# cure-lab/MotionCraft

Hardware: AMD Instinct MI355X
Metric: sampled SMPL-X frames/sec (196-frame seq, 1000-step DDPM) (higher is better)
Workload: dtype f32

## Files before the change

include/motioncraft_amd.h:

```cpp
#ifndef MOTIONCRAFT_AMD_H
#define MOTIONCRAFT_AMD_H
#include <stdint.h>

#ifdef __cplusplus
extern "C" {
#endif

#define MC_OK 0
#define MC_ERR_ARG 1
#define MC_ERR_HIP 2
#define MC_ERR_STATE 3
#define MC_ERR_NOCONV 4

typedef struct mc_model mc_model;
typedef struct mc_ctx mc_ctx;

typedef struct mc_model_config {
    int32_t input_feats;
    int32_t max_seq_len;
    int32_t latent_dim;
    int32_t num_parts;
    int32_t num_layers;
    int32_t ffn_dim;
    int32_t time_embed_dim;
// ... 137 lines not shown
int mc_op_temporal_attention(const float* mf_dev, const float* tf_dev, const float* mask_dev, float* yt_dev, int32_t b0, int32_t nb,
                             int32_t B, int32_t T, int32_t Nt, int32_t H, int32_t L, int32_t form, int32_t skip_text,
                             const int32_t* twin_flag_dev, void* stream);
enum { MC_ENC_ATTN_LAYER = 0,
       MC_ENC_ATTN_SMALL = 1,
       MC_ENC_ATTN_STREAM = 2 };
int mc_op_enc_ln(const float* x_dev, const float* gamma_dev, const float* beta_dev, float* y_dev, int64_t rows, int32_t L, float eps,
                 int32_t relu, void* stream);
int mc_op_enc_embed_tokens(const int32_t* ids_dev, const float* emb_dev, const float* pos_dev, float* x_dev, int64_t rows, int32_t S,
                           int32_t d, int32_t vocab, void* stream);
int mc_op_enc_attention(const float* qkv_dev, const uint8_t* valid_dev, float* out_dev, int32_t B, int32_t S, int32_t d, int32_t heads,
                        int32_t causal, int32_t form, void* stream);
enum { MC_GM_PLAIN = 0, MC_GM_ENC = 4 };
typedef struct mc_gemm_strided {
    const float* a_dev; int64_t lda, a_gstride;
    const float* w_dev; int64_t ldw, w_gstride;
    const float* bias_dev; int64_t b_gstride;
    float* c_dev; int64_t ldc, c_gstride;
    const float* res_dev; int64_t ldr, r_gstride;
    const float* add_dev; int64_t ld_add, dup_rows;
    int32_t add_mod, act, act_after_res, M, N, K;
} mc_gemm_strided;
int mc_op_gemm_strided(int32_t mode, int32_t groups, const mc_gemm_strided* args, void* stream);
int mc_op_bigru_steps(const float* gi_dev, const float* whh_dev, const float* bhh_dev, float* h_dev, const int32_t* lens_dev,
                      int32_t len_div, int32_t B, int32_t S, int32_t H, int32_t s0, int32_t steps, void* stream);
int mc_op_conv1d_k4s2(const float* x_dev, int64_t ldx, const float* w_tapmajor_dev, const float* bias_dev, float* y_padded_dev, int32_t B,
                      int32_t T, int32_t C, int32_t Cp, int32_t O, float slope, void* stream);
int mc_op_sampler_update(const float* x_t_dev, const float* out_text_dev, const float* out_none_dev,
                         const float* noise_dev, float* x_prev_dev, float* x0_dev, int64_t n,
                         const mc_step_coefs* coefs, void* stream);
int mc_op_sampler_multistep(const float* x_t_dev, const float* out_text_dev, const float* out_none_dev, float* x0_hist_dev,
                            float* x_prev_dev, float* x0_dev, int64_t n, const mc_step_coefs* coefs, void* stream);
int mc_op_gemm_tail_rows(const float* h_dev, const float* a_dev, const float* w_dev, const float* bias_dev, float* c_dev, float* c2_dev,
                         int32_t M, int32_t N, int32_t K, const mc_step_coefs* coefs_host, int32_t T, int32_t variant, void* stream);
int mc_op_sampler_rows(const float* x_t_dev, const float* out_text_dev, const float* out_none_dev, const float* noise_dev,
                       float* x0_hist_dev, float* x_prev_dev, float* x0_dev, int32_t B, int32_t TC, const mc_step_coefs* coefs_host,
                       void* stream);
int mc_op_sampler_edit_rows(const float* x_t_dev, const float* out_text_dev, const float* out_none_dev, const float* noise_dev,
                            const float* gt_noise_dev, const float* gt_dev, const uint8_t* keep_dev, const uint64_t* seeds_host,
                            const uint64_t* draw_host, float* x0_hist_dev, float* x_prev_dev, float* x0_dev, int32_t B, int32_t TC,
                            const mc_step_coefs* coefs_host, void* stream);
int mc_op_sampler_seam(const float* x_t_dev, const float* out_text_dev, const float* out_none_dev, const float* noise_dev, uint64_t seed,
                       uint64_t draw, float* x0_hist_dev, float* x_prev_dev, float* x0_dev, int32_t B, int32_t T, int32_t C,
                       int32_t overlap, const int32_t* first_frame_host, const float* weight_host, const mc_step_coefs* coefs,
                       void* stream);

// ... 229 lines not shown
```

motioncraft_amd/csrc/mc_ctx.h:

```cpp
#pragma once
#include <map>
#include <mutex>
#include <string>
#include <vector>

#include "../../include/motioncraft_amd.h"
#include "mc_common.h"
#include "mc_gemm.h"
#include "mc_kernels.h"
#include "mc_chain.h"
#include "mc_half.h"
#include "mc_options.h"
#include "mc_params.h"

struct mc_model {
    mc_model_config cfg;
    ParamStore params{""};
    std::map<std::string, HalfW> half;
    std::mutex half_mu;
    size_t half_bytes = 0;
    bool finalized = false;
    int Cp = 0;
};

// ... 4 lines not shown

struct LayerW {
    const float *norm_g, *norm_b, *tnorm_g, *tnorm_b, *wsm;
    MoeW mm, tm;
    const float *dyn_g, *dyn_b, *qkv_w, *qkv_b;
    const float *ca_film_w, *ca_film_b, *ca_ln_g, *ca_ln_b, *ca_out_w, *ca_out_b;
    const float *ffn_w1, *ffn_b1, *ffn_w2, *ffn_b2;
    const float *ffn_film_w, *ffn_film_b, *ffn_ln_g, *ffn_ln_b, *ffn_out_w, *ffn_out_b;
    const float *before_w = nullptr, *before_b = nullptr, *after_w = nullptr, *after_b = nullptr;
    HalfW h_ca_out, h_ffn_out, h_fc1, h_fc2, h_w1, h_w2, h_after, h_proj, h_qkv;
};

struct ProfRec { hipEvent_t e0 = nullptr, e1 = nullptr; long rows = 0; };

struct mc_ctx {
    mc_model* m = nullptr;
    McOptions opt{};
    int B = 0, T = 0, S = 0, maxS = 0;
    long N = 0, rows = 0, Ntxt = 0;
    std::vector<LayerW> lw;
    const float *enc_w, *enc_b, *seq_emb, *time_w0, *time_b0, *time_w2, *time_b2, *dec_w, *dec_b;
    const float *dec_wf = nullptr, *dec_bf = nullptr;
    float *dec_cat_w = nullptr, *dec_cat_b = nullptr;
    const float *ctrl_in_w = nullptr, *ctrl_in_b = nullptr;
    int NLA = 0;
    float *hc = nullptr, *cb = nullptr, *cenc = nullptr;
    bool have_ctrl = false;
    std::vector<void*> allocs;
    int64_t bytes = 0;
    float *h, *z, *proj, *hbuf, *y2, *mf, *qkv, *ys, *yt, *a, *z2, *fh, *out2, *xpad;
    float* a_tail = nullptr;
    size_t hbuf_cap = 0;
    size_t hbuf_floats = 0;
    bool cnt_clean = false;
    long led_nsrc = 0, led_gsplit = 0;
    float *xfn, *tf;
    const float* mask = nullptr;
    float* mask_own = nullptr;
    int* t_orig;
    float *te, *e1, *emb, *semb, *ss;
    RouteBufs rb;
    int device = 0;
    int coop_reserved = 0;
    bool prof_on = false;
    std::vector<ProfRec> prof;
    bool have_cond = false;
// ... 82 lines not shown
```

motioncraft_amd/csrc/mc_gemm.h:

```cpp
#pragma once
#include <hip/hip_runtime.h>
#include "mc_options.h"
#include "../../include/motioncraft_amd.h"

enum { GM_PLAIN = MC_GM_PLAIN, GM_EXP1 = 1, GM_EXP2 = 2, GM_COMB = 3, GM_ENC = MC_GM_ENC };

enum : int {
    kTuneStaging = 1 << 0,
    kTuneDma = 1 << 4,
    kTuneWp = 1 << 5,
    kTuneNoXcd = 1 << 6,
    kTuneSmallXcd = 1 << 8,
    kTuneEncWp = 1 << 9,
    kTuneTail2 = 1 << 10,
    kTuneBits = kTuneStaging | kTuneDma | kTuneWp | kTuneNoXcd | kTuneSmallXcd | kTuneEncWp | kTuneTail2,
    kTuneDefault = kTuneBits & ~kTuneNoXcd,
};
static_assert(kTuneDefault == 1841, "the default tune bits are public ABI");

struct GemmArgs {
    const float* A = nullptr;
    long lda = 0;
    int a_col = 0;
    long a_gstride = 0;
    const float* W = nullptr;
    long ldw = 0;
    long w_gstride = 0;
    const float* bias = nullptr;
    long b_gstride = 0;
    float* C = nullptr;
    long ldc = 0;
    int c_col = 0;
    long c_gstride = 0;
    const float* R = nullptr;
    long ldr = 0;
    long r_gstride = -1;
    int act = 0;
    int act_after_res = 0;
    const float* add = nullptr;
    int add_mod = 1;
    long ld_add = 0;
    long dup_rows = 0;
    int M = 0, N = 0, K = 0;
    const int* tile_group = nullptr;
    const int* tile_row0 = nullptr;
    const int* tile_nrows = nullptr;
    const int* num_tiles = nullptr;
    const int* src_row = nullptr;
    const int* dst_row = nullptr;
    const float* comb_w = nullptr;
    int small_tile_n = 0;
    int wp_grid = 0;
    int tune = -1;
};

inline void mc_gemm_opts(const McOptions& o, GemmArgs& g) {
    g.tune = (int)o.gemm_tune;
    g.small_tile_n = o.small_tile_n ? (int)o.small_tile_n : -1;
    g.wp_grid = o.gemm_wp_grid > 0 ? (int)o.gemm_wp_grid : -1;
}

inline double mc_cu_load(long workgroups) {
    const long n = (workgroups + 255) / 256;
    return (1.45 * (double)(n / 2) + (double)(n % 2));
}

int mc_device_cus();
int mc_launch_gemm(int mode, const GemmArgs& g, int groups, int max_tiles, hipStream_t stream);
int mc_launch_gemm_small(const GemmArgs& g, hipStream_t stream, int groups = 1);

struct TailArgs {
    const float* H = nullptr;
    const float* Af = nullptr;
    long half = 0, lda = 0;
    const float* W = nullptr;
    long ldw = 0, w_gstride = 0;
    const float* bias = nullptr;
    long b_gstride = 0;
    float* C = nullptr;
    float* C2 = nullptr;
    long ldc = 0;
    int M = 0, N = 0, K = 0;
    float wc = 1.f, wu = 0.f;
    int rows_T = 0;
    const float* coef_table = nullptr;
    const int* step_ptr = nullptr;
    long coef_stride = 0;
    int tune = -1;
// ... 6 lines not shown
```

motioncraft_amd/csrc/mc_gemm.hip:

```cpp
#include "mc_common.h"
#include "mc_gemm.h"

namespace {

constexpr int BM = 128, BN = 128, BK = 32, LD = BK + 4;

struct Stage {
    long aoff[4], woff[4];
    bool aok[4], wok[4];
    float cw0[4], cw1[4];
};

template <int MODE, bool GUARD>
__device__ __forceinline__ void load_tile(const GemmArgs& g, const float* __restrict__ Ab, const float* __restrict__ Wb,
                                          const Stage& st, int k, f32x4 (&ra)[4], f32x4 (&rb)[4]) {
    const bool kin = !GUARD || k < g.K;
#pragma unroll
    for (int i = 0; i < 4; ++i) {
        f32x4 v = {0.f, 0.f, 0.f, 0.f};
        if ((!GUARD || st.aok[i]) && kin) {
            if constexpr (MODE == GM_COMB) {
                f32x4 y0 = {0.f, 0.f, 0.f, 0.f}, y1 = {0.f, 0.f, 0.f, 0.f};
                if (st.cw0[i] != 0.f) y0 = *reinterpret_cast<const f32x4*>(Ab + st.aoff[i] + k);
                if (st.cw1[i] != 0.f) y1 = *reinterpret_cast<const f32x4*>(Ab + st.aoff[i] + g.lda + k);
// ... 312 lines not shown
        const float* At = As + buf * BM * BK + (wm * 64 + frow) * BK;
        const float* Bt = Bs + buf * BN * BK + (wn * 64 + frow) * BK;
        Frag f0 = ld_frag(At, Bt, 0);
        Frag f1 = ld_frag(At, Bt, 1);
        __builtin_amdgcn_sched_barrier(0);
        mma(f0);
        f0 = ld_frag(At, Bt, 2);
        __builtin_amdgcn_sched_barrier(0);
        mma(f1);
        f1 = ld_frag(At, Bt, 3);
        __builtin_amdgcn_sched_barrier(0);
        mma(f0);
        mma(f1);
        __syncthreads();
    }
    if (g.act == ACT_GELU) epilogue_vec<GM_PLAIN, false, ACT_GELU>(g, 0, row0, BM, tn, wm, wn, lane, acc);
    else if (g.act == ACT_SILU) epilogue_vec<GM_PLAIN, false, ACT_SILU>(g, 0, row0, BM, tn, wm, wn, lane, acc);
    else if (g.act == ACT_NONE) epilogue_vec<GM_PLAIN, false, ACT_NONE>(g, 0, row0, BM, tn, wm, wn, lane, acc);
    else epilogue_vec<GM_PLAIN, false, ACT_LRELU>(g, 0, row0, BM, tn, wm, wn, lane, acc);
}

constexpr int WBK = 16, WSTAGE = 128 * WBK;

__global__ __launch_bounds__(256, 2) void gemm_wp_k(GemmArgs g) {
    __shared__ __attribute__((aligned(16))) float smem[4 * 2 * WSTAGE];
    const int tid = threadIdx.x, lane = tid & 63, wave = tid >> 6;
    const int wm = wave >> 1, wn = wave & 1;
    const int ntn = g.N / BN, ntiles = (g.M / BM) * ntn;
    const int wave_u = __builtin_amdgcn_readfirstlane(wave);
    float* wbase = smem + wave_u * 2 * WSTAGE;
    const unsigned lds0 = (unsigned)(size_t)wbase;
    const int dr = lane >> 2, dc = ((lane & 3) ^ ((dr >> 2) & 3)) * 4;
    const int frow = lane & 31, hf = lane >> 5, sw = (frow >> 2) & 3;
    const float* Ab = g.A + g.a_col;
    const float* Wb = g.W;
    const float* __restrict__ Rb = g.R ? g.R + g.c_col : nullptr;
    float* __restrict__ Cb = g.C + g.c_col;
    const int nk = g.K / WBK;
    struct Frag { f32x4 a0, a1, b0, b1; };
    auto ld_frag = [&](int st, int j) {
        const float* S = wbase + st * WSTAGE + frow * WBK + ((2 * j + hf) ^ sw) * 4;
        Frag f;
        f.a0 = *reinterpret_cast<const f32x4*>(S);
        f.a1 = *reinterpret_cast<const f32x4*>(S + 32 * WBK);
        f.b0 = *reinterpret_cast<const f32x4*>(S + 64 * WBK);
        f.b1 = *reinterpret_cast<const f32x4*>(S + 96 * WBK);
        return f;
    };
    for (int t = blockIdx.x; t < ntiles; t += gridDim.x) {
        const int bid = (g.tune & kTuneNoXcd) ? t : xcd_remap(t, ntiles);
        const int tm = bid / ntn, tn = bid % ntn;
        const int row0 = tm * BM;
        unsigned voa[4], vow[4];
#pragma unroll
        for (int q = 0; q < 4; ++q) {
            voa[q] = (unsigned)(((long)(row0 + wm * 64 + 16 * q + dr) * g.lda + dc) * 4);
            vow[q] = (unsigned)(((long)(tn * BN + wn * 64 + 16 * q + dr) * g.ldw + dc) * 4);
        }
        auto issue_q = [&](int kt, int st, int q) {
            const unsigned l = lds0 + st * WSTAGE * 4;
            dma16(voa[q], Ab + kt * WBK, l + q * 1024);
            dma16(vow[q], Wb + kt * WBK, l + 4096 + q * 1024);
        };
        f32x16 acc[2][2];
#pragma unroll
        for (int mi = 0; mi < 2; ++mi)
#pragma unroll
            for (int ni = 0; ni < 2; ++ni)
#pragma unroll
                for (int r = 0; r < 16; ++r) acc[mi][ni][r] = 0.f;
        auto mma2 = [&](const Frag& f, int i0) {
#pragma unroll
            for (int i = i0; i < i0 + 2; ++i) {
                acc[0][0] = __builtin_amdgcn_mfma_f32_32x32x2f32(f.b0[i], f.a0[i], acc[0][0], 0, 0, 0);
                acc[0][1] = __builtin_amdgcn_mfma_f32_32x32x2f32(f.b1[i], f.a0[i], acc[0][1], 0, 0, 0);
                acc[1][0] = __builtin_amdgcn_mfma_f32_32x32x2f32(f.b0[i], f.a1[i], acc[1][0], 0, 0, 0);
                acc[1][1] = __builtin_amdgcn_mfma_f32_32x32x2f32(f.b1[i], f.a1[i], acc[1][1], 0, 0, 0);
            }
        };
#pragma unroll
        for (int q = 0; q < 4; ++q) issue_q(0, 0, q);
        asm volatile("s_waitcnt vmcnt(0)" ::: "memory");
        Frag f0 = ld_frag(0, 0);
        auto ktile = [&](int kt) {
            const int st = kt & 1;
            const bool more = kt + 1 < nk;
            Frag f1 = ld_frag(st, 1);
            __builtin_amdgcn_sched_barrier(0);
            mma2(f0, 0);
            if (more) { issue_q(kt + 1, st ^ 1, 0); issue_q(kt + 1, st ^ 1, 1); }
            __builtin_amdgcn_sched_barrier(0);
            mma2(f0, 2);
            if (more) { issue_q(kt + 1, st ^ 1, 2); issue_q(kt + 1, st ^ 1, 3); }
            __builtin_amdgcn_sched_barrier(0);
            mma2(f1, 0);
            if (more) {
                asm volatile("s_waitcnt vmcnt(0)" ::: "memory");
                f0 = ld_frag(st ^ 1, 0);
            }
            __builtin_amdgcn_sched_barrier(0);
            mma2(f1, 2);
        };
        const int npre = nk > 2 ? nk - 2 : 0;
        for (int kt = 0; kt < npre; ++kt) ktile(kt);
        f32x4 rv[2][2][4], bv[2][4];
#pragma unroll
        for (int ni = 0; ni < 2; ++ni)
#pragma unroll
            for (int q = 0; q < 4; ++q) {
                const int n = tn * BN + wn * 64 + ni * 32 + 8 * q + 4 * hf;
                bv[ni][q] = g.bias ? *reinterpret_cast<const f32x4*>(g.bias + n) : f32x4{0.f, 0.f, 0.f, 0.f};
#pragma unroll
                for (int mi = 0; mi < 2; ++mi) {
                    const long m = row0 + wm * 64 + mi * 32 + frow;
                    rv[mi][ni][q] = Rb ? *reinterpret_cast<const f32x4*>(Rb + m * g.ldr + n) : f32x4{0.f, 0.f, 0.f, 0.f};
                    if (g.add) rv[mi][ni][q] = *reinterpret_cast<const f32x4*>(g.add + (m % g.add_mod) * g.ld_add + n);
// ... 597 lines not shown
    MC_LAUNCH_CHECK();
    return MC_OK;
}

int mc_launch_gemm(int mode, const GemmArgs& g0, int groups, int max_tiles, hipStream_t stream) {
    GemmArgs g = g0;
    if (int r = resolve_opts(g)) return r;
    const int ntn = cdiv(g.N, BN);
    int ntm = (mode == GM_EXP1 || mode == GM_EXP2) ? max_tiles : cdiv(g.M, BM);
    if (ntm <= 0 || ntn <= 0) return MC_OK;
    if (mode != GM_ENC) MC_REQUIRE(g.K % 4 == 0 && g.lda % 4 == 0 && g.ldw % 4 == 0, "gemm: K/lda/ldw must be multiples of 4");
    if (mode == GM_ENC && (g.add || g.dup_rows))
        MC_REQUIRE(g.N % 4 == 0 && g.ldc % 4 == 0 && g.c_col % 4 == 0 && g.c_gstride % 4 == 0 && (!g.add || g.ld_add % 4 == 0) &&
                       (!g.R || (g.ldr % 4 == 0 && (g.r_gstride < 0 || g.r_gstride % 4 == 0))),
                   "gemm: an add table or duplicate rows need 16-byte aligned output rows (N=%d ldc=%ld)", g.N, g.ldc);
    dim3 grid(ntm * ntn, groups > 0 ? groups : 1, 1);
    const bool vec_out = (g.ldc % 4 == 0) && (g.c_col % 4 == 0) && (!g.R || g.ldr % 4 == 0);
    const bool wp_ok = (g.tune & kTuneWp) && g.K % WBK == 0 && (long)g.M * g.lda * 4 < (1L << 32) && (long)g.N * g.ldw * 4 < (1L << 32);
    const bool enc_fast = mode == GM_ENC && (g.tune & kTuneEncWp) && wp_ok && !g.R && g.add && g.ld_add % 4 == 0 && g.act == ACT_NONE;
    if ((g.tune & kTuneDma) && (mode == GM_PLAIN || enc_fast) && groups <= 1 && g.M % BM == 0 && g.N % BN == 0 && (g.K % BK == 0 || enc_fast) &&
        g.lda % 4 == 0 && g.ldw % 4 == 0 && g.a_col % 4 == 0 && vec_out && g.act != ACT_QUICKGELU && !g.act_after_res &&
        (enc_fast || (!g.add && !g.dup_rows))) {
        if (wp_ok) {
            const int persistent = g.wp_grid > 0 ? g.wp_grid : (int)grid.x;
            MC_LEDGER("gemm_wp_k", dim3(grid.x < persistent ? grid.x : persistent), 2.0 * g.M * g.N * g.K);
            hipLaunchKernelGGL(gemm_wp_k, dim3(grid.x < persistent ? grid.x : persistent), dim3(256), 0, stream, g);
        } else {
            MC_LEDGER("gemm_dma_k", grid, 2.0 * g.M * g.N * g.K);
            hipLaunchKernelGGL(gemm_dma_k, grid, dim3(256), 0, stream, g);
        }
        MC_LAUNCH_CHECK();
        return MC_OK;
    }
    if (mc_ledger_on) {
        char name[24];
        snprintf(name, sizeof(name), "gemm_k<%d>", mode);
        const double rows = (mode == GM_EXP1 || mode == GM_EXP2) ? (double)ntm * BM : (double)g.M;
        MC_LEDGER(name, grid, 2.0 * rows * g.N * g.K * (groups > 0 ? groups : 1));
    }
    switch (mode) {
        case GM_PLAIN: hipLaunchKernelGGL(gemm_k<GM_PLAIN>, grid, dim3(256), 0, stream, g); break;
        case GM_EXP1: hipLaunchKernelGGL(gemm_k<GM_EXP1>, grid, dim3(256), 0, stream, g); break;
        case GM_EXP2: hipLaunchKernelGGL(gemm_k<GM_EXP2>, grid, dim3(256), 0, stream, g); break;
        case GM_COMB: hipLaunchKernelGGL(gemm_k<GM_COMB>, grid, dim3(256), 0, stream, g); break;
        case GM_ENC: hipLaunchKernelGGL(gemm_k<GM_ENC>, grid, dim3(256), 0, stream, g); break;
        default: mc_set_error("bad gemm mode %d", mode); return MC_ERR_ARG;
    }
    MC_LAUNCH_CHECK();
    return MC_OK;
}

int mc_device_cus() {
    static int v = 0;
    if (v <= 0) {
        int dev = 0;
        hipDeviceProp_t prop;
        if (hipGetDevice(&dev) == hipSuccess && hipGetDeviceProperties(&prop, dev) == hipSuccess) v = prop.multiProcessorCount;
        if (v <= 0) v = 256;
    }
    return v;
}

static int tail2_grid(const TailArgs& g, int tune, int* per_wave_out) {
    const int ncb = cdiv(g.N, 16);
    const long nblocks = (long)cdiv(g.M, 16) * ncb;
    if (!(tune & kTuneTail2) || !g.C2 || ncb > T2_MAXCB || g.K < 3 * T2_BK || g.K % T2_BK) return 0;
    int G = mc_device_cus();
    if (nblocks < (long)G * 16) G = (int)(nblocks / 16) > 0 ? (int)(nblocks / 16) : 1;
    else G *= (int)cdiv(nblocks, (long)G * 66);
    const int nmax = (int)cdiv(nblocks, (long)G);
    const int per_wave = cdiv(nmax, 4);
// ... 62 lines not shown
```

motioncraft_amd/csrc/mc_model.hip:

```cpp
#include "mc_ctx.h"

#include <cstring>

namespace {

template <class T>
int ws_alloc(mc_ctx* c, T** p, size_t n) {
    void* d = nullptr;
    size_t bytes = (n * sizeof(T) + 255) & ~(size_t)255;
    if (bytes == 0) bytes = 256;
    MC_HIP(hipMalloc(&d, bytes));
    c->allocs.push_back(d);
    c->bytes += (int64_t)bytes;
    *p = (T*)d;
    return MC_OK;
}

int bind_moe(const mc_model* m, const std::string& pre, int din, int dout, int seq_rows, MoeW* w) {
    const int64_t E = m->cfg.num_experts;
    w->din = din;
    w->dout = dout;
    return m->params.bind({{&w->emb, pre + "emb", (int64_t)seq_rows * din},       {&w->gate_w, pre + "gate_w", 256 * din},
                           {&w->gate_b, pre + "gate_b", 256},                      {&w->sim_n, pre + "sim_n", 256 * E},
                           {&w->sim_nT, pre + "sim_nT", 32 * 256},                 {&w->scale, pre + "scale", 1},
// ... 33 lines not shown
            if ((r = ps.bind({{&w.after_w, p + "after_w", DD}, {&w.after_b, p + "after_b", D}}))) return r;
        }
        if ((r = ps.bind({{&w.norm_g, p + "norm.g", L},                         {&w.norm_b, p + "norm.b", L},
                          {&w.tnorm_g, p + "text_norm.g", g.text_latent_dim},   {&w.tnorm_b, p + "text_norm.b", g.text_latent_dim},
                          {&w.wsm, p + "body_wsm", H * H}})))
            return r;
        if ((r = bind_moe(m, p + "mm.", L, 4 * L, g.max_seq_len * H, &w.mm))) return r;
        if ((r = bind_moe(m, p + "tm.", g.text_latent_dim, 2 * L, g.max_text_len, &w.tm))) return r;
        if ((r = ps.bind({{&w.dyn_g, p + "dyn.norm.g", L},                      {&w.dyn_b, p + "dyn.norm.b", L},
                          {&w.qkv_w, p + "dyn.qkv_w", 3 * L * L},               {&w.qkv_b, p + "dyn.qkv_b", 3 * L},
                          {&w.ca_film_w, p + "ca.film_w", (int64_t)2 * D * Te}, {&w.ca_film_b, p + "ca.film_b", 2 * D},
                          {&w.ca_ln_g, p + "ca.ln_g", D},                       {&w.ca_ln_b, p + "ca.ln_b", D},
                          {&w.ca_out_w, p + "ca.out_w", DD},                    {&w.ca_out_b, p + "ca.out_b", D},
                          {&w.ffn_w1, p + "ffn.w1", (int64_t)H * F * L},        {&w.ffn_b1, p + "ffn.b1", H * F},
                          {&w.ffn_w2, p + "ffn.w2", (int64_t)H * L * F},        {&w.ffn_b2, p + "ffn.b2", H * L},
                          {&w.ffn_film_w, p + "ffn.film_w", (int64_t)2 * D * Te}, {&w.ffn_film_b, p + "ffn.film_b", 2 * D},
                          {&w.ffn_ln_g, p + "ffn.ln_g", D},                     {&w.ffn_ln_b, p + "ffn.ln_b", D},
                          {&w.ffn_out_w, p + "ffn.out_w", DD},                  {&w.ffn_out_b, p + "ffn.out_b", D}})))
            return r;
    }
    return MC_OK;
}

int build_ctx_weights(mc_ctx* c) {
    if (!c->dec_wf) return MC_OK;
    const mc_model_config& g = c->m->cfg;
    const int D = g.latent_dim * g.num_parts;
    const size_t wn = (size_t)g.input_feats * D, bn = (size_t)g.input_feats;
    int rr;
    if ((rr = ws_alloc(c, &c->dec_cat_w, 2 * wn)) != MC_OK || (rr = ws_alloc(c, &c->dec_cat_b, 2 * bn)) != MC_OK) return rr;
    MC_HIP(hipMemcpy(c->dec_cat_w, c->dec_w, wn * sizeof(float), hipMemcpyDeviceToDevice));
    MC_HIP(hipMemcpy(c->dec_cat_w + wn, c->dec_wf, wn * sizeof(float), hipMemcpyDeviceToDevice));
    MC_HIP(hipMemcpy(c->dec_cat_b, c->dec_bf, bn * sizeof(float), hipMemcpyDeviceToDevice));
    MC_HIP(hipMemset(c->dec_cat_b + bn, 0, bn * sizeof(float)));
    return MC_OK;
}

int half_weight(mc_model* m, const std::string& name, long rows, int K, bool chain, HalfW* out) {
    std::lock_guard<std::mutex> lock(m->half_mu);
    auto it = m->half.find(name);
    if (it != m->half.end()) { *out = it->second; return MC_OK; }
    const float* src = nullptr;
    int r = m->params.get(name, (int64_t)rows * K, &src);
    if (r != MC_OK) return r;
    mc_half* hi = nullptr;
    MC_HIP(hipMalloc((void**)&hi, sizeof(mc_half) * 2 * (size_t)rows * K));
    mc_half* lo = hi + (size_t)rows * K;
    r = chain ? mc_launch_split_f16_chainperm(src, hi, lo, rows, K, nullptr) : mc_launch_split_f16(src, hi, lo, rows * K, nullptr);
    if (r != MC_OK) { (void)hipFree(hi); return r; }
    MC_HIP(hipStreamSynchronize(nullptr));
    const HalfW h{hi, lo};
    m->half[name] = h;
// ... 39 lines not shown

struct OptionDef {
    const char *key, *env, *env_alt;
    long McOptions::*field;
    long dflt;
    std::string (*check)(long v);
    int (*hook)(mc_ctx* c, long& v);
};

std::string check_chain(long v) {
    const long bad = v & ~kChainDefault;
    const int b = bad ? __builtin_ctzl((unsigned long)bad) : 0;
    return !bad ? "" : "chain bit " + std::to_string(b) + (b < kChainBits ? " is retired (DESIGN.md section 5)" : " is not defined");
}
std::string check_tune(long v) {
    const long bad = v & ~(long)kTuneBits;
    return !bad ? "" : v < 0 ? "gemm_tune: a bit mask (>= 0)" : "gemm_tune bit " + std::to_string(__builtin_ctzl(bad)) + " is not defined";
}
int chain_hook(mc_ctx* c, long& v) {
    const int L = c->m->cfg.latent_dim;
    c->hbuf_floats = ((v >> kChainMlp) & 1) && mc_mlp_supported(L, 4 * L) ? c->hbuf_cap : 0;
    return MC_OK;
}
int route_coop_hook(mc_ctx* c, long& v) {
    if (!v) {
        if (c->coop_reserved) { mc_route_coop_release(c->device, c->coop_reserved); c->coop_reserved = 0; }
    } else if (!c->opt.route_coop) {
        const int nwg = coop_grid_needed(c);
        MC_REQUIRE(nwg == 0 || mc_route_coop_reserve(c->device, nwg), "route_coop: the cooperative routing grid cannot be reserved on this device");
        c->coop_reserved = nwg;
        v = nwg > 0;
    }
    return MC_OK;
}

const OptionDef kOptions[] = {
    {"chain", "MC_CHAIN", nullptr, &McOptions::chain, kChainDefault, check_chain, chain_hook},
    {"small_gemm_rows", "MC_SMALL_GEMM_ROWS", nullptr, &McOptions::small_gemm_rows, 5600},
    {"split_rows_expert", "MC_SPLIT_ROWS_EXPERT", nullptr, &McOptions::split_rows_expert, 2048},
    {"split_rows_sffn", "MC_SPLIT_ROWS_SFFN", nullptr, &McOptions::split_rows_sffn, 8192},
    {"temporal_split", "MC_TEMPORAL_SPLIT", nullptr, &McOptions::temporal_split, 96},
    {"big_tokens", "MC_BIG_TOKENS", nullptr, &McOptions::big_tokens, 65536},
    {"rowchain_split", "MC_ROWCHAIN_SPLIT", nullptr, &McOptions::rowchain_split, 20480},
    {"gemm_tune", "MC_GEMM_TUNE", nullptr, &McOptions::gemm_tune, kTuneDefault, check_tune},
    {"small_tile_n", "MC_SMALL_TILE_N", nullptr, &McOptions::small_tile_n, 0,
     [](long v) -> std::string { return v == 0 || v == 48 || v == 64 || v == 96 ? "" : "small_tile_n: 0 (per-launch choice), 48, 64 or 96"; }},
    {"gemm_wp_grid", "MC_GEMM_WP_GRID", nullptr, &McOptions::gemm_wp_grid, 512},
    {"half_min_rows", "MC_HALF_MIN_ROWS", nullptr, &McOptions::half_min_rows, 512},
    {"gate_small", "MC_GATE_SMALL", nullptr, &McOptions::gate_small, 12000},
    {"split_expert", "MC_SPLIT_EXPERT", nullptr, &McOptions::split_expert, 0},
    {"split_sffn", "MC_SPLIT_SFFN", nullptr, &McOptions::split_sffn, 0},
    {"route_reg", "MC_ROUTE_REG", nullptr, &McOptions::route_reg, 1},
    {"route_coop", "MC_ROUTE_COOP", nullptr, &McOptions::route_coop, 1, nullptr, route_coop_hook},
    {"route_small", "MC_ROUTE_SMALL_CTX", "MC_ROUTE_SMALL", &McOptions::route_small, 20480,
     [](long v) -> std::string { return v >= 0 && v <= 131072 ? "" : "route_small: 0 .. 131072 pairs (the one-workgroup kernels hold at most 131072)"; }},
    {"route_early", "MC_ROUTE_EARLY", nullptr, &McOptions::route_early, 1,
     [](long v) -> std::string { return v == 0 || v == 1 ? "" : "route_early: 0 or 1"; }},
    {"route_per", nullptr, nullptr, &McOptions::route_per, 0,
     [](long v) -> std::string { return v == 0 || v == 10 || v == 16 ? "" : "route_per: 0 (default), 10 or 16"; }},
    {"dbg_delay_us", nullptr, nullptr, &McOptions::dbg_delay_us, 0,
     [](long v) -> std::string { return v >= -100000 && v <= 100000 ? "" : "dbg_delay_us: -100000 .. 100000"; }},
};

int seed_options(McOptions& o) {
    for (const OptionDef& d : kOptions) {
        const char *var = nullptr, *e = nullptr;
        for (const char* v : {d.env, d.env_alt})
            if (v && !e && (e = getenv(v))) var = v;
        const std::string why = e && d.check ? d.check(atol(e)) : "";
        MC_REQUIRE(why.empty(), "%s=%s: %s", var, e, why.c_str());
// ... 1022 lines not shown
int mc_op_gemm(const float* a, const float* w, const float* bias, const float* res, float* cdev, int32_t M, int32_t N,
               int32_t K, int32_t ldw, int32_t act, void* stream) {
    MC_REQUIRE(a && w && cdev && M > 0 && N > 0 && K > 0 && K % 4 == 0 && ldw % 4 == 0 && ldw >= K, "bad gemm args");
    return dense(nullptr, a, K, w, ldw, bias, res, N, cdev, N, M, N, K, act, (hipStream_t)stream);
}

int mc_op_gemm_strided(int32_t mode, int32_t groups, const mc_gemm_strided* a, void* stream) {
    MC_REQUIRE(a && (mode == GM_PLAIN || mode == GM_ENC) && groups >= 1, "gemm_strided: mode %d (0 plain, 4 encoder), groups %d", mode, groups);
    MC_REQUIRE(a->a_dev && a->w_dev && a->c_dev && a->M > 0 && a->N > 0 && a->K > 0 && a->lda > 0 && a->ldc >= a->N && a->ldw >= a->K &&
                   a->ldw % 4 == 0 && a->add_mod >= 1 && a->dup_rows >= 0 && (!a->res_dev || a->ldr >= a->N) && (!a->add_dev || a->ld_add >= a->N),
               "bad gemm_strided args");
    GemmArgs g;
    g.A = a->a_dev; g.lda = a->lda; g.a_gstride = a->a_gstride;
    g.W = a->w_dev; g.ldw = a->ldw; g.w_gstride = a->w_gstride;
    g.bias = a->bias_dev; g.b_gstride = a->b_gstride;
    g.C = a->c_dev; g.ldc = a->ldc; g.c_gstride = a->c_gstride;
    g.R = a->res_dev; g.ldr = a->ldr; g.r_gstride = a->r_gstride;
    g.act = a->act; g.act_after_res = a->act_after_res;
    g.add = a->add_dev; g.add_mod = a->add_mod; g.ld_add = a->ld_add; g.dup_rows = a->dup_rows;
    g.M = a->M; g.N = a->N; g.K = a->K;
    return mc_launch_gemm(mode, g, groups, 0, (hipStream_t)stream);
}

static int gemm_f16_op(GemmHArgs g, const float* w, const float* bias, const float* res, float* cdev, int M, int N, int K, bool split, hipStream_t s) {
    mc_half* planes = nullptr;
    MC_HIP(hipMalloc((void**)&planes, sizeof(mc_half) * 2 * (size_t)N * K));
    int r = mc_launch_split_f16(w, planes, planes + (size_t)N * K, (long)N * K, s);
    if (r == MC_OK) {
        g.Wh = planes; g.Wl = planes + (size_t)N * K; g.bias = bias; g.R = res; g.ldr = N; g.C = cdev; g.ldc = N;
        g.M = M; g.N = N; g.K = K;
        r = mc_launch_gemm_h(g, split, s);
    }
    (void)hipStreamSynchronize(s);
    (void)hipFree(planes);
    return r;
}

int mc_op_gemm_f16(const float* a, const float* w, const float* bias, const float* res, float* cdev, int32_t M, int32_t N,
                   int32_t K, int32_t split, void* stream) {
    MC_REQUIRE(a && w && cdev && M > 0 && N > 0 && K > 0, "bad gemm args");
    GemmHArgs g;
    g.A = a; g.lda = K;
    return gemm_f16_op(g, w, bias, res, cdev, M, N, K, split != 0, (hipStream_t)stream);
}

int mc_op_gemm_f16_planes(const void* a_hi, const void* a_lo, const float* w, const float* bias, const float* res, float* cdev, int32_t M,
// ... 348 lines not shown
```

motioncraft_amd/csrc/mc_step.hip:

```cpp
#include "mc_ctx.h"

bool use_half(const mc_ctx* c) { return c->prec != MC_PREC_F32 && c->rows > c->opt.half_min_rows; }
static const HalfW* half_planes(const mc_ctx* c, const HalfW* hw) { return hw && hw->hi && use_half(c) ? hw : nullptr; }
static bool split3(const mc_ctx* c) { return c->prec == MC_PREC_F16X3; }

static bool twin_aliased(const mc_ctx* c, bool twin) { return twin && !c->no_alias; }
static TwinAlias twin_alias(const mc_ctx* c, bool twin, bool tokens) {
    return twin_aliased(c, twin) ? TwinAlias{mc_route_split_flag_ptr(c->rb), (tokens ? c->N : c->rows) / 2} : TwinAlias();
}

template <class Args>
static void set_tile_map(const mc_ctx* c, int group, Args& a) {
    const long to = (long)group * c->rb.max_tiles;
    a.tile_group = c->rb.tile_group + to; a.tile_row0 = c->rb.tile_row0 + to; a.tile_nrows = c->rb.tile_nrows + to;
    a.num_tiles = mc_route_num_tiles_ptr(c->rb, group);
}

static int dbg_hold(const mc_ctx* c, hipStream_t pos, hipStream_t neg) {
    const long us = c->opt.dbg_delay_us;
    return us == 0 ? MC_OK : mc_launch_spin((us > 0 ? us : -us) * 100, us > 0 ? pos : neg);
}

int dense(const mc_ctx* c, const float* A, long lda, const float* W, long ldw, const float* bias, const float* R, long ldr,
          float* C, long ldc, long M, int N, int K, int act, hipStream_t s) {
// ... 531 lines not shown
    return layer_rows_tail(c, i, hs, step, twin, half, half, c->side, nullptr, p.stagger ? c->ev_stag : nullptr);
}

int denoise_impl(mc_ctx* c, const float* x_t, int32_t step, float* out2_dev, int32_t stop_after, void* stream, const SeedArgs* seed) {
    MC_REQUIRE(c && x_t, "null argument");
    MC_REQUIRE(c->have_cond, "mc_ctx_set_condition not called");
    MC_REQUIRE(step >= 0 && step < c->S, "step_index %d outside the %d-step schedule", step, c->S);
    if (c->graph_mode) step = 0;
    if (c->rows_mode) step = 0;
    hipStream_t s = (hipStream_t)stream;
    const mc_model_config& g = c->m->cfg;
    const int L = g.latent_dim, H = g.num_parts, D = L * H, C = g.input_feats;
    const long BT = (long)c->B * c->T;
    int r;
    if ((r = pick_side_stream(c, s))) return r;
    {
        const bool padded = c->xpad_ready && !seed;
        c->xpad_ready = false;
        if (seed) { if ((r = mc_launch_pad_rows_seeded(const_cast<float*>(x_t), c->xpad, BT, C, c->m->Cp, *seed, s))) return r; }
        else if (!padded && (r = mc_launch_pad_rows(x_t, c->xpad, BT, C, c->m->Cp, s))) return r;
        GemmArgs e;
        mc_gemm_opts(c->opt, e);
        e.A = c->xpad; e.lda = c->m->Cp;
        e.W = c->enc_w; e.ldw = c->m->Cp; e.bias = c->enc_b;
        e.add = c->seq_emb; e.add_mod = c->T; e.ld_add = D;
        e.C = c->h; e.ldc = D; e.dup_rows = BT;
        e.M = (int)BT; e.N = D; e.K = c->m->Cp;
        if (BT <= c->opt.small_gemm_rows && D % 64 == 0 && c->m->Cp % 32 == 0) { if ((r = mc_launch_gemm_small(e, s))) return r; }
        else if ((r = mc_launch_gemm(GM_ENC, e, 1, 0, s))) return r;
    }
    const int nl = stop_after >= 0 ? (stop_after < g.num_layers ? stop_after : g.num_layers) : g.num_layers;
    c->no_alias = stop_after >= 0 && stop_after < g.num_layers;
    const int NC = c->have_ctrl ? g.num_ctrl_layers : 0;
    const bool fused = chain_on(c, kChainGate) && chain_on(c, kChainRowchain) && mc_mlp_supported(L, 32);
    const bool two_groups = c->side && chain_on(c, kChainTwoStreams) && c->N > c->opt.big_tokens && fused;
    auto by_group = [&](auto&& fn) -> int {
        if (!two_groups) return fn(0L, c->rows, s);
        if (int e = fn(0L, BT, s)) return e;
        return fn(BT, BT, c->side);
    };
    for (int i = 0; i < nl; ++i) {
        if (i >= 1 && i <= NC) {
            const int j = i - 1, slot = g.num_layers + j;
            if (j == 0) {
                if ((r = by_group([&](long r0, long n, hipStream_t sk) {
                         return mc_launch_add_rows(c->hc + r0 * D, c->h + r0 * D, c->cb + r0 * D, nullptr, n, D, sk); })))
                    return r;
// ... 131 lines not shown
```

Measured before the change: 670.1.

## Skip all-zero K blocks in encoder GEMM via precomputed per-tile schedule

Scans the encoder weight matrix on the host for 16-wide K blocks that are all zero in each 128-column tile, and builds a table that gives each persistent workgroup its tiles and K-block bitmasks. Tiles are assigned to workgroups greedily by cost (longest first). A templated path of the persistent GEMM kernel walks only the nonzero K blocks. This is aimed at the zero-padded input features (Cp > C) and any structural zeros in the encoder weight. In exchange it adds host setup work and a device sync when the grid option changes, and the speedup depends on how sparse the weight actually is.

Result: no change. 672.6 (median of 6 runs) (+0.4%).

```diff
diff --git a/include/motioncraft_amd.h b/include/motioncraft_amd.h
--- a/include/motioncraft_amd.h
+++ b/include/motioncraft_amd.h
@@ -183,6 +183,8 @@
     int32_t add_mod, act, act_after_res, M, N, K;
 } mc_gemm_strided;
 int mc_op_gemm_strided(int32_t mode, int32_t groups, const mc_gemm_strided* args, void* stream);
+int mc_op_gemm_kmask(const float* w_host, int32_t N, int32_t K, int64_t ldw, uint64_t* masks_host);
+int mc_op_gemm_enc_sparse(const mc_gemm_strided* args, int32_t wp_grid, uint64_t* masks_host, void* stream);
 int mc_op_bigru_steps(const float* gi_dev, const float* whh_dev, const float* bhh_dev, float* h_dev, const int32_t* lens_dev,
                       int32_t len_div, int32_t B, int32_t S, int32_t H, int32_t s0, int32_t steps, void* stream);
 int mc_op_conv1d_k4s2(const float* x_dev, int64_t ldx, const float* w_tapmajor_dev, const float* bias_dev, float* y_padded_dev, int32_t B,
diff --git a/motioncraft_amd/csrc/mc_ctx.h b/motioncraft_amd/csrc/mc_ctx.h
--- a/motioncraft_amd/csrc/mc_ctx.h
+++ b/motioncraft_amd/csrc/mc_ctx.h
@@ -50,6 +50,8 @@
     const float *enc_w, *enc_b, *seq_emb, *time_w0, *time_b0, *time_w2, *time_b2, *dec_w, *dec_b;
     const float *dec_wf = nullptr, *dec_bf = nullptr;
     float *dec_cat_w = nullptr, *dec_cat_b = nullptr;
+    int* enc_ktab = nullptr;
+    int enc_ktab_ntm = 0, enc_ktab_grid = 0;
     const float *ctrl_in_w = nullptr, *ctrl_in_b = nullptr;
     int NLA = 0;
     float *hc = nullptr, *cb = nullptr, *cenc = nullptr;
diff --git a/motioncraft_amd/csrc/mc_gemm.h b/motioncraft_amd/csrc/mc_gemm.h
--- a/motioncraft_amd/csrc/mc_gemm.h
+++ b/motioncraft_amd/csrc/mc_gemm.h
@@ -13,10 +13,11 @@
     kTuneSmallXcd = 1 << 8,
     kTuneEncWp = 1 << 9,
     kTuneTail2 = 1 << 10,
-    kTuneBits = kTuneStaging | kTuneDma | kTuneWp | kTuneNoXcd | kTuneSmallXcd | kTuneEncWp | kTuneTail2,
+    kTuneEncSparse = 1 << 11,
+    kTuneBits = kTuneStaging | kTuneDma | kTuneWp | kTuneNoXcd | kTuneSmallXcd | kTuneEncWp | kTuneTail2 | kTuneEncSparse,
     kTuneDefault = kTuneBits & ~kTuneNoXcd,
 };
-static_assert(kTuneDefault == 1841, "the default tune bits are public ABI");
+static_assert(kTuneDefault == 3889, "the default tune bits are public ABI");
 
 struct GemmArgs {
     const float* A = nullptr;
@@ -49,6 +50,8 @@
     const int* src_row = nullptr;
     const int* dst_row = nullptr;
     const float* comb_w = nullptr;
+    const int* ktab = nullptr;
+    int ktab_ntm = 0, ktab_grid = 0;
     int small_tile_n = 0;
     int wp_grid = 0;
     int tune = -1;
@@ -64,6 +67,13 @@
     const long n = (workgroups + 255) / 256;
     return (1.45 * (double)(n / 2) + (double)(n % 2));
 }
+
+constexpr int kKtabEpilogue = 4;
+inline int mc_ktab_ints(int ntn, int ntm, int grid) { return 4 * ntm * ntn + grid + 1; }
+inline int mc_wp_grid(int ntiles, int wp_grid) { return wp_grid > 0 && wp_grid < ntiles ? wp_grid : ntiles; }
+void mc_gemm_kmask_host(const float* w_host, int N, int K, long ldw, unsigned long long* masks);
+void mc_gemm_ktab_host(const unsigned long long* masks, int ntn, int ntm, int grid, int* tab);
+int mc_gemm_ktab_upload(const float* w_dev, int N, int K, long ldw, int ntm, int grid, int* tab_dev, unsigned long long* masks_out);
 
 int mc_device_cus();
 int mc_launch_gemm(int mode, const GemmArgs& g, int groups, int max_tiles, hipStream_t stream);
diff --git a/motioncraft_amd/csrc/mc_gemm.hip b/motioncraft_amd/csrc/mc_gemm.hip
--- a/motioncraft_amd/csrc/mc_gemm.hip
+++ b/motioncraft_amd/csrc/mc_gemm.hip
@@ -1,5 +1,12 @@
 #include "mc_common.h"
 #include "mc_gemm.h"
+
+#include <algorithm>
+#include <cstring>
+#include <functional>
+#include <queue>
+#include <utility>
+#include <vector>
 
 namespace {
 
@@ -358,6 +365,7 @@
 
 constexpr int WBK = 16, WSTAGE = 128 * WBK;
 
+template <bool KL>
 __global__ __launch_bounds__(256, 2) void gemm_wp_k(GemmArgs g) {
     __shared__ __attribute__((aligned(16))) float smem[4 * 2 * WSTAGE];
     const int tid = threadIdx.x, lane = tid & 63, wave = tid >> 6;
@@ -372,7 +380,6 @@
     const float* Wb = g.W;
     const float* __restrict__ Rb = g.R ? g.R + g.c_col : nullptr;
     float* __restrict__ Cb = g.C + g.c_col;
-    const int nk = g.K / WBK;
     struct Frag { f32x4 a0, a1, b0, b1; };
     auto ld_frag = [&](int st, int j) {
         const float* S = wbase + st * WSTAGE + frow * WBK + ((2 * j + hf) ^ sw) * 4;
@@ -383,8 +390,25 @@
         f.b1 = *reinterpret_cast<const f32x4*>(S + 96 * WBK);
         return f;
     };
-    for (int t = blockIdx.x; t < ntiles; t += gridDim.x) {
-        const int bid = (g.tune & kTuneNoXcd) ? t : xcd_remap(t, ntiles);
+    const int4* __restrict__ sched = reinterpret_cast<const int4*>(g.ktab);
+    int t = blockIdx.x, tend = ntiles, tstep = gridDim.x;
+    int e_tile = 0, e_lo = 0, e_hi = 0;
+    if constexpr (KL) {
+        const int* start = g.ktab + 4 * ntiles;
+        t = start[blockIdx.x], tend = start[blockIdx.x + 1], tstep = 1;
+        const int4 e = sched[t < tend ? t : 0];
+        e_tile = __builtin_amdgcn_readfirstlane(e.x), e_lo = __builtin_amdgcn_readfirstlane(e.y), e_hi = __builtin_amdgcn_readfirstlane(e.z);
+    }
+    for (; t < tend; t += tstep) {
+        int bid, nk = g.K / WBK;
+        unsigned long long kmask = 0;
+        if constexpr (KL) {
+            bid = e_tile;
+            kmask = (unsigned long long)(unsigned)e_lo | ((unsigned long long)(unsigned)e_hi << 32);
+            nk = __builtin_popcountll(kmask);
+        } else {
+            bid = (g.tune & kTuneNoXcd) ? t : xcd_remap(t, ntiles);
+        }
         const int tm = bid / ntn, tn = bid % ntn;
         const int row0 = tm * BM;
         unsigned voa[4], vow[4];
@@ -393,10 +417,14 @@
             voa[q] = (unsigned)(((long)(row0 + wm * 64 + 16 * q + dr) * g.lda + dc) * 4);
             vow[q] = (unsigned)(((long)(tn * BN + wn * 64 + 16 * q + dr) * g.ldw + dc) * 4);
         }
-        auto issue_q = [&](int kt, int st, int q) {
+        auto kcol = [&](int kt) {
+            if constexpr (KL) { const int k = __builtin_ctzll(kmask); kmask &= kmask - 1; return k * WBK; }
+            else return kt * WBK;
+        };
+        auto issue_q = [&](int kc, int st, int q) {
             const unsigned l = lds0 + st * WSTAGE * 4;
-            dma16(voa[q], Ab + kt * WBK, l + q * 1024);
-            dma16(vow[q], Wb + kt * WBK, l + 4096 + q * 1024);
+            dma16(voa[q], Ab + kc, l + q * 1024);
+            dma16(vow[q], Wb + kc, l + 4096 + q * 1024);
         };
         f32x16 acc[2][2];
 #pragma unroll
@@ -414,20 +442,28 @@
                 acc[1][1] = __builtin_amdgcn_mfma_f32_32x32x2f32(f.b1[i], f.a1[i], acc[1][1], 0, 0, 0);
             }
         };
-#pragma unroll
-        for (int q = 0; q < 4; ++q) issue_q(0, 0, q);
+        Frag f0 = {};
+        if (!KL || nk > 0) {
+            const int kc = kcol(0);
+#pragma unroll
+            for (int q = 0; q < 4; ++q) issue_q(kc, 0, q);
+        }
+        int4 e_next = {0, 0, 0, 0};
+        if constexpr (KL) e_next = sched[t + 1 < tend ? t + 1 : t];
         asm volatile("s_waitcnt vmcnt(0)" ::: "memory");
-        Frag f0 = ld_frag(0, 0);
+        if constexpr (KL) e_tile = __builtin_amdgcn_readfirstlane(e_next.x), e_lo = __builtin_amdgcn_readfirstlane(e_next.y), e_hi = __builtin_amdgcn_readfirstlane(e_next.z);
+        if (!KL || nk > 0) f0 = ld_frag(0, 0);
         auto ktile = [&](int kt) {
             const int st = kt & 1;
             const bool more = kt + 1 < nk;
+            const int kc = more ? kcol(kt + 1) : 0;
             Frag f1 = ld_frag(st, 1);
             __builtin_amdgcn_sched_barrier(0);
             mma2(f0, 0);
-            if (more) { issue_q(kt + 1, st ^ 1, 0); issue_q(kt + 1, st ^ 1, 1); }
+            if (more) { issue_q(kc, st ^ 1, 0); issue_q(kc, st ^ 1, 1); }
             __builtin_amdgcn_sched_barrier(0);
             mma2(f0, 2);
-            if (more) { issue_q(kt + 1, st ^ 1, 2); issue_q(kt + 1, st ^ 1, 3); }
+            if (more) { issue_q(kc, st ^ 1, 2); issue_q(kc, st ^ 1, 3); }
             __builtin_amdgcn_sched_barrier(0);
             mma2(f1, 0);
             if (more) {
@@ -1071,9 +1107,11 @@
         g.lda % 4 == 0 && g.ldw % 4 == 0 && g.a_col % 4 == 0 && vec_out && g.act != ACT_QUICKGELU && !g.act_after_res &&
         (enc_fast || (!g.add && !g.dup_rows))) {
         if (wp_ok) {
-            const int persistent = g.wp_grid > 0 ? g.wp_grid : (int)grid.x;
-            MC_LEDGER("gemm_wp_k", dim3(grid.x < persistent ? grid.x : persistent), 2.0 * g.M * g.N * g.K);
-            hipLaunchKernelGGL(gemm_wp_k, dim3(grid.x < persistent ? grid.x : persistent), dim3(256), 0, stream, g);
+            const int persistent = mc_wp_grid((int)grid.x, g.wp_grid);
+            const bool sparse = enc_fast && (g.tune & kTuneEncSparse) && g.ktab && g.ktab_ntm == ntm && g.ktab_grid == persistent && g.K / WBK <= 64;
+            MC_LEDGER("gemm_wp_k", dim3(persistent), 2.0 * g.M * g.N * g.K);
+            if (sparse) hipLaunchKernelGGL(gemm_wp_k<true>, dim3(persistent), dim3(256), 0, stream, g);
+            else hipLaunchKernelGGL(gemm_wp_k<false>, dim3(persistent), dim3(256), 0, stream, g);
         } else {
             MC_LEDGER("gemm_dma_k", grid, 2.0 * g.M * g.N * g.K);
             hipLaunchKernelGGL(gemm_dma_k, grid, dim3(256), 0, stream, g);
@@ -1096,6 +1134,62 @@
         default: mc_set_error("bad gemm mode %d", mode); return MC_ERR_ARG;
     }
     MC_LAUNCH_CHECK();
+    return MC_OK;
+}
+
+void mc_gemm_kmask_host(const float* w, int N, int K, long ldw, unsigned long long* masks) {
+    for (int tn = 0; tn < N / BN; ++tn) {
+        unsigned long long m = 0;
+        for (int r = tn * BN; r < (tn + 1) * BN; ++r)
+            for (int k = 0; k < K; ++k) {
+                unsigned bits;
+                memcpy(&bits, w + (long)r * ldw + k, sizeof(bits));
+                if (bits << 1) m |= 1ull << (k / WBK);
+            }
+        masks[tn] = m;
+    }
+}
+void mc_gemm_ktab_host(const unsigned long long* masks, int ntn, int ntm, int grid, int* tab) {
+    const int ntiles = ntm * ntn;
+    auto cost = [&](int tile) { return __builtin_popcountll(masks[tile % ntn]) + kKtabEpilogue; };
+    std::vector<int> tiles(ntiles);
+    for (int i = 0; i < ntiles; ++i) tiles[i] = i;
+    std::stable_sort(tiles.begin(), tiles.end(), [&](int a, int b) { return cost(a) > cost(b); });
+    std::priority_queue<std::pair<long, int>, std::vector<std::pair<long, int>>, std::greater<std::pair<long, int>>> heap;
+    for (int b = 0; b < grid; ++b) heap.push({0L, b});
+    std::vector<std::vector<int>> mine(grid);
+    for (int tile : tiles) {
+        auto [load, b] = heap.top();
+        heap.pop();
+        mine[b].push_back(tile);
+        heap.push({load + cost(tile), b});
+    }
+    int *sched = tab, *start = tab + 4 * ntiles, n = 0;
+    for (int b = 0; b < grid; ++b) {
+        start[b] = n;
+        for (int tile : mine[b]) {
+            const unsigned long long m = masks[tile % ntn];
+            sched[4 * n] = tile;
+            sched[4 * n + 1] = (int)(unsigned)(m & 0xffffffffull);
+            sched[4 * n + 2] = (int)(unsigned)(m >> 32);
+            sched[4 * n + 3] = 0;
+            ++n;
+        }
+    }
+    start[grid] = n;
+}
+int mc_gemm_ktab_upload(const float* w_dev, int N, int K, long ldw, int ntm, int grid, int* tab_dev, unsigned long long* masks_out) {
+    MC_REQUIRE(w_dev && tab_dev && N > 0 && N % BN == 0 && K > 0 && K % WBK == 0 && K / WBK <= 64 && ldw >= K && ntm > 0 && grid > 0 && grid <= ntm * (N / BN),
+               "gemm zero map: N=%d K=%d ldw=%ld, %d row tiles on %d workgroups", N, K, ldw, ntm, grid);
+    const int ntn = N / BN;
+    std::vector<float> w((size_t)N * K);
+    MC_HIP(hipMemcpy2D(w.data(), (size_t)K * sizeof(float), w_dev, (size_t)ldw * sizeof(float), (size_t)K * sizeof(float), (size_t)N, hipMemcpyDeviceToHost));
+    std::vector<unsigned long long> masks(ntn);
+    mc_gemm_kmask_host(w.data(), N, K, K, masks.data());
+    std::vector<int> tab(mc_ktab_ints(ntn, ntm, grid));
+    mc_gemm_ktab_host(masks.data(), ntn, ntm, grid, tab.data());
+    MC_HIP(hipMemcpy(tab_dev, tab.data(), tab.size() * sizeof(int), hipMemcpyHostToDevice));
+    if (masks_out) memcpy(masks_out, masks.data(), masks.size() * sizeof(masks[0]));
     return MC_OK;
 }
 
diff --git a/motioncraft_amd/csrc/mc_model.hip b/motioncraft_amd/csrc/mc_model.hip
--- a/motioncraft_amd/csrc/mc_model.hip
+++ b/motioncraft_amd/csrc/mc_model.hip
@@ -79,12 +79,28 @@
     return MC_OK;
 }
 
+int build_enc_ktab(mc_ctx* c, long wp_grid) {
+    const mc_model_config& g = c->m->cfg;
+    const int D = g.latent_dim * g.num_parts, Cp = c->m->Cp;
+    const long BT = (long)c->B * c->T;
+    if (D % 128 || BT % 128 || Cp % 16 || Cp / 16 > 64) return MC_OK;
+    const int ntn = D / 128, ntm = (int)(BT / 128), grid = mc_wp_grid(ntm * ntn, wp_grid > 0 ? (int)wp_grid : -1);
+    int rr;
+    if (!c->enc_ktab && (rr = ws_alloc(c, &c->enc_ktab, (size_t)mc_ktab_ints(ntn, ntm, ntm * ntn))) != MC_OK) return rr;
+    c->enc_ktab_ntm = c->enc_ktab_grid = 0;
+    if ((rr = mc_gemm_ktab_upload(c->enc_w, D, Cp, Cp, ntm, grid, c->enc_ktab, nullptr)) != MC_OK) return rr;
+    c->enc_ktab_ntm = ntm;
+    c->enc_ktab_grid = grid;
+    return MC_OK;
+}
+
 int build_ctx_weights(mc_ctx* c) {
-    if (!c->dec_wf) return MC_OK;
     const mc_model_config& g = c->m->cfg;
     const int D = g.latent_dim * g.num_parts;
+    int rr;
+    if ((rr = build_enc_ktab(c, c->opt.gemm_wp_grid)) != MC_OK) return rr;
+    if (!c->dec_wf) return MC_OK;
     const size_t wn = (size_t)g.input_feats * D, bn = (size_t)g.input_feats;
-    int rr;
     if ((rr = ws_alloc(c, &c->dec_cat_w, 2 * wn)) != MC_OK || (rr = ws_alloc(c, &c->dec_cat_b, 2 * bn)) != MC_OK) return rr;
     MC_HIP(hipMemcpy(c->dec_cat_w, c->dec_w, wn * sizeof(float), hipMemcpyDeviceToDevice));
     MC_HIP(hipMemcpy(c->dec_cat_w + wn, c->dec_wf, wn * sizeof(float), hipMemcpyDeviceToDevice));
@@ -170,6 +186,10 @@
     c->hbuf_floats = ((v >> kChainMlp) & 1) && mc_mlp_supported(L, 4 * L) ? c->hbuf_cap : 0;
     return MC_OK;
 }
+int wp_grid_hook(mc_ctx* c, long& v) {
+    MC_HIP(hipDeviceSynchronize());
+    return build_enc_ktab(c, v);
+}
 int route_coop_hook(mc_ctx* c, long& v) {
     if (!v) {
         if (c->coop_reserved) { mc_route_coop_release(c->device, c->coop_reserved); c->coop_reserved = 0; }
@@ -193,7 +213,7 @@
     {"gemm_tune", "MC_GEMM_TUNE", nullptr, &McOptions::gemm_tune, kTuneDefault, check_tune},
     {"small_tile_n", "MC_SMALL_TILE_N", nullptr, &McOptions::small_tile_n, 0,
      [](long v) -> std::string { return v == 0 || v == 48 || v == 64 || v == 96 ? "" : "small_tile_n: 0 (per-launch choice), 48, 64 or 96"; }},
-    {"gemm_wp_grid", "MC_GEMM_WP_GRID", nullptr, &McOptions::gemm_wp_grid, 512},
+    {"gemm_wp_grid", "MC_GEMM_WP_GRID", nullptr, &McOptions::gemm_wp_grid, 512, nullptr, wp_grid_hook},
     {"half_min_rows", "MC_HALF_MIN_ROWS", nullptr, &McOptions::half_min_rows, 512},
     {"gate_small", "MC_GATE_SMALL", nullptr, &McOptions::gate_small, 12000},
     {"split_expert", "MC_SPLIT_EXPERT", nullptr, &McOptions::split_expert, 0},
@@ -1262,6 +1282,44 @@
     return mc_launch_gemm(mode, g, groups, 0, (hipStream_t)stream);
 }
 
+int mc_op_gemm_kmask(const float* w_host, int32_t N, int32_t K, int64_t ldw, uint64_t* masks_host) {
+    MC_REQUIRE(w_host && masks_host && N > 0 && N % 128 == 0 && K > 0 && K % 16 == 0 && K <= 1024 && ldw >= K, "gemm_kmask: N=%d K=%d ldw=%ld", N, K, (long)ldw);
+    static_assert(sizeof(uint64_t) == sizeof(unsigned long long), "mask words");
+    mc_gemm_kmask_host(w_host, N, K, ldw, (unsigned long long*)masks_host);
+    return MC_OK;
+}
+
+int mc_op_gemm_enc_sparse(const mc_gemm_strided* a, int32_t wp_grid, uint64_t* masks_host, void* stream) {
+    MC_REQUIRE(a && a->a_dev && a->w_dev && a->c_dev && a->add_dev && !a->res_dev && a->act == ACT_NONE && a->M > 0 && a->M % 128 == 0 && a->N > 0 &&
+                   a->N % 128 == 0 && a->K > 0 && a->K % 16 == 0 && a->K <= 1024 && a->lda >= a->K && a->lda % 4 == 0 && a->ldw >= a->K && a->ldw % 4 == 0 &&
+                   a->ldc >= a->N && a->ldc % 4 == 0 && a->ld_add >= a->N && a->ld_add % 4 == 0 && a->add_mod >= 1 && a->dup_rows >= 0,
+               "gemm_enc_sparse: full 128 x 128 tiles, K %% 16 == 0, K <= 1024, 16-byte aligned rows, a table, no residual, no activation");
+    const McOptions* o = mc_process_options();
+    if (!o) return MC_ERR_ARG;
+    GemmArgs g;
+    mc_gemm_opts(*o, g);
+    g.tune |= kTuneDma | kTuneWp | kTuneEncWp | kTuneEncSparse;
+    if (wp_grid > 0) g.wp_grid = wp_grid;
+    g.A = a->a_dev; g.lda = a->lda;
+    g.W = a->w_dev; g.ldw = a->ldw;
+    g.bias = a->bias_dev;
+    g.C = a->c_dev; g.ldc = a->ldc;
+    g.add = a->add_dev; g.add_mod = a->add_mod; g.ld_add = a->ld_add; g.dup_rows = a->dup_rows;
+    g.M = a->M; g.N = a->N; g.K = a->K;
+    MC_REQUIRE((long)g.M * g.lda * 4 < (1L << 32) && (long)g.N * g.ldw * 4 < (1L << 32), "gemm_enc_sparse: operands beyond 4 GB");
+    const int ntn = g.N / 128, ntm = g.M / 128;
+    int* tab = nullptr;
+    g.ktab_ntm = ntm;
+    g.ktab_grid = mc_wp_grid(ntm * ntn, g.wp_grid);
+    MC_HIP(hipMalloc((void**)&tab, sizeof(int) * mc_ktab_ints(ntn, ntm, g.ktab_grid)));
+    g.ktab = tab;
+    int r = mc_gemm_ktab_upload(g.W, g.N, g.K, g.ldw, ntm, g.ktab_grid, tab, (unsigned long long*)masks_host);
+    if (r == MC_OK) r = mc_launch_gemm(GM_ENC, g, 1, 0, (hipStream_t)stream);
+    (void)hipStreamSynchronize((hipStream_t)stream);
+    (void)hipFree(tab);
+    return r;
+}
+
 static int gemm_f16_op(GemmHArgs g, const float* w, const float* bias, const float* res, float* cdev, int M, int N, int K, bool split, hipStream_t s) {
     mc_half* planes = nullptr;
     MC_HIP(hipMalloc((void**)&planes, sizeof(mc_half) * 2 * (size_t)N * K));
diff --git a/motioncraft_amd/csrc/mc_step.hip b/motioncraft_amd/csrc/mc_step.hip
--- a/motioncraft_amd/csrc/mc_step.hip
+++ b/motioncraft_amd/csrc/mc_step.hip
@@ -577,7 +577,7 @@
         GemmArgs e;
         mc_gemm_opts(c->opt, e);
         e.A = c->xpad; e.lda = c->m->Cp;
-        e.W = c->enc_w; e.ldw = c->m->Cp; e.bias = c->enc_b;
+        e.W = c->enc_w; e.ldw = c->m->Cp; e.bias = c->enc_b; e.ktab = c->enc_ktab; e.ktab_ntm = c->enc_ktab_ntm; e.ktab_grid = c->enc_ktab_grid;
         e.add = c->seq_emb; e.add_mod = c->T; e.ld_add = D;
         e.C = c->h; e.ldc = D; e.dup_rows = BT;
         e.M = (int)BT; e.N = D; e.K = c->m->Cp;
```
